# schatty/oprl

Measured on AMD Instinct MI355X. Metric: learner gradient steps/sec, DDPG batch=256 walker-walk, higher is better.
Workload: dtype f32 (exact-fp32 MFMA)

## Files before the change

oprl_amd/csrc/fused_ddpg.hip:

```cpp
#include <cstddef>
#include <mutex>
#include <type_traits>
#include "kernels.h"
#include "philox.h"
#include "replay_index.h"
#include "batch_rows.h"
#include "slice_head.h"
#include "tp4.h"
#include "dw_body.h"
#include "dw_tile_x2.h"

namespace oprl { constexpr bool kDwTileX2 = true; constexpr bool kMergedTile64 = true; }

namespace oprl {


__device__ __forceinline__ bool cluster_on_one_xcd(const DdpgArgs& A) {
  const int xcc = __builtin_amdgcn_s_getreg((3 << 11) | 20) & 15;
  return A.xcd_local != 0 && ((int)gridDim.x & 7) == 0 && xcc == ((int)blockIdx.x & 7);
}
__global__ void k_xcc_probe(int* out) {
  if (threadIdx.x == 0) out[blockIdx.y * gridDim.x + blockIdx.x] = __builtin_amdgcn_s_getreg((3 << 11) | 20) & 15;
}

// ... 893 lines not shown
  long long* trace;
  const float* pb1_32 = nullptr;
  unsigned mS = 0, mA = 0;
};
template <class P, class KA = DwKArgs, bool PF = true, bool GE = false>
__device__ __forceinline__ int ddpg_phase2m_body(const DdpgArgs& A, const KA* D, int by_in, const PassCtx& cx) {
  static_assert((P::kX2 || GE) && kDwTileX2, "the merged phase 2: PrecX2 learners; with the unit-seed rows (k_ddpg_chain) every arithmetic");
  extern __shared__ __attribute__((aligned(16))) float smem[];
  using LY = FusedLds<256>;
  constexpr int HB = kR * kWL4;
  constexpr int NMC = 8;
  const int B = A.B, S = A.S, Ad = A.A, tid = threadIdx.x;
  const int slice = blockIdx.x, row0 = slice * kR;
  const int y = by_in < 0 ? (int)blockIdx.y : by_in;
  const int yP = NMC, yT = yP + ((PF && A.prefetch_next) ? 1 : 0);
  if (y >= yT) {
    const int tile = (y - yT) * (int)gridDim.x + slice;
    if (tile >= dw_total(*D)) return -1;
    if (A.whole) {
      wait_flags(A.w_flags, 4 * (int)gridDim.x, cx.epoch, A.err, (KERN_PHASE2 << 8) | SITE_DW_GATE);
      __syncthreads();
    }
    return tile;
  }
  float* xa = smem + LY::xa;
  if (PF && y == yP) {
    float* xb = smem + LY::xb;
    float* rS = smem + LY::misc;
    float* dS = rS + kR;
    int* meta = reinterpret_cast<int*>(dS + 2 * kR);
    int* endsS = reinterpret_cast<int*>(smem + LY::misc + 96);
    load_batch(A.next, row0, B, S, Ad, xa, xb, rS, dS, meta, endsS);
    __syncthreads();
    store_rows(xa, kX0Ld, const_cast<float*>(A.next.s), S, S, row0, B);
    store_rows(xb, kX0Ld, const_cast<float*>(A.next.s2), S, S, row0, B);
    for (int idx = tid; idx < kR * Ad; idx += kThreads) {
      const int row = idx / Ad, col = idx - row * Ad, gr = row0 + row;
      if (gr < B) const_cast<float*>(A.next.a)[(size_t)gr * Ad + col] = xa[row * kX0Ld + S + col];
    }
    if (tid < kR && row0 + tid < B) {
      const_cast<float*>(A.next.r)[row0 + tid] = rS[tid];
      const_cast<float*>(A.next.d)[row0 + tid] = dS[tid];
    }
    return -1;
  }
  float* h1 = smem + LY::h;
  float* h2 = h1 + HB;
  float* g2 = h2 + HB;
  float* Wl = g2 + HB;
  float* outS = smem + LY::out;
  float* auxS = smem + LY::aux;
  float* duS = smem + LY::aux2;
  float* scr = smem + LY::scr;
  float* w3s = smem + LY::misc + 96;
  static_assert(2 * HB >= 2 * 8 * 512, "the shard fits the two spare hidden buffers");
  static_assert(kMaxEnds >= kDuLd * 256, "W3 fits the ends table's area");
  Tp tp{y, NMC, A.xbuf + (size_t)slice * kTpStages * A.xnc * kTpBlk, cx.tag, 0,
        A.err, KERN_PHASE2 << 8, A.debug_expire == (int)SITE_CLUSTER ? 0 : kTpSpin};
  tp.local = GE && cluster_on_one_xcd(A);
  const bool lead = tp.c == 0;
  const int c = tp.c;
  const int lane = tid & 63, wave = tid >> 6, i = lane & 15, kk = lane >> 4;
  long long* const trace = cx.trace;
  int n_stamp = 0;
  auto stamp = [&]() {
    if (kTraceOn && trace != nullptr && (tid & 63) == 0 && (tid == 0 || slice == 0) && lead && n_stamp < kTraceStamps) {
      const int slot = tid == 0 ? slice : 16 + (tid >> 6);
      long long* tr = trace + ((size_t)slot * kTraceStamps + n_stamp) * 2;
      tr[0] = (long long)__builtin_readcyclecounter();
      tr[1] = (long long)wall_clock64();
    }
    ++n_stamp;
  };
  stamp();
  const Tp3Store nostore{nullptr, nullptr, nullptr, nullptr, 0};
  BiasOv cbo;
  if (A.whole) {
    wait_flags(A.w_flags, 4 * (int)gridDim.x, cx.epoch, A.err, (KERN_PHASE2 << 8) | SITE_DW_GATE);
    __syncthreads();
  }
  stamp();
  {
    const float* p0 = A.aX[0]; const float* p3 = A.pi; const int ld0 = A.aldx0;
    asm volatile("" :: "s"(p0), "s"(p3), "s"(ld0));
  }
  const float* wsrc = ((P::kBf16 && cx.pb1_32 != nullptr) ? cx.pb1_32 : A.actor.pb[1]) + (size_t)c * 2 * 16 * 256;
  f32x4 wv[2];
#pragma unroll
  for (int q = 0; q < 2; ++q) wv[q] = ld4c(wsrc + ((size_t)q * kThreads + tid) * 4);
  const int hr = tid >> 6, hc = (tid & 63) * 4;
  f32x4 hv = f32x4{0.f, 0.f, 0.f, 0.f};
  if (row0 + hr < B) hv = ld4c(A.aX[2] + (size_t)(row0 + hr) * kW4 + hc);
  f32x4 w3q = f32x4{0.f, 0.f, 0.f, 0.f};
  if ((tid >> 6) < Ad) w3q = ld4c(cx.w3 + (size_t)tid * 4);
  const int et = (tid >> 8) & 1, er = (tid >> 4) & 15, ec = tid & 15;
  float m1 = 0.f;
  if (!GE && tid < 512 && row0 + er < B) m1 = ldc(A.aX[1] + (size_t)(row0 + er) * kW4 + 32 * c + 16 * et + ec);
  f32x4 gm1 = f32x4{0.f, 0.f, 0.f, 0.f};
  if constexpr (GE) {
#pragma unroll
    for (int r = 0; r < 4; ++r)
      if (row0 + 4 * kk + r < B) gm1[r] = ldc(A.aX[1] + (size_t)(row0 + 4 * kk + r) * kW4 + 32 * c + 16 * (wave & 1) + i);
  }
  const int rs_ = GE ? row_div(tid, cx.mS) : tid / S, cs_ = tid - rs_ * S;
  const bool oks = tid < kR * S && row0 + rs_ < B;
  const float vs = oks ? ldc(A.aX[0] + (size_t)(row0 + rs_) * A.aldx0 + cs_) : 0.f;
  const int tid2 = tid + kThreads;
  const int rs2_ = GE ? row_div(tid2, cx.mS) : tid2 / S, cs2_ = tid2 - rs2_ * S;
  const bool oks2 = tid2 < kR * S && row0 + rs2_ < B;
  const float vs2 = oks2 ? ldc(A.aX[0] + (size_t)(row0 + rs2_) * A.aldx0 + cs2_) : 0.f;
  const int rp_ = GE ? row_div(tid, cx.mA) : tid / Ad, cp_ = tid - rp_ * Ad;
  const bool okp = tid < kR * Ad && row0 + rp_ < B;
  const float vp = okp ? ldc(A.pi + (size_t)(row0 + rp_) * Ad + cp_) : 0.f;
  lds_zero(xa, kR * kX0Ld);
  lds_zero(auxS, kR * kOutLd);
  __syncthreads();
  if (tid < kR * S) xa[rs_ * kX0Ld + cs_] = vs;
  if (tid2 < kR * S) xa[rs2_ * kX0Ld + cs2_] = vs2;
  if (tid < kR * Ad) xa[rp_ * kX0Ld + S + cp_] = vp;
#pragma unroll
  for (int q = 0; q < 2; ++q) *reinterpret_cast<f32x4*>(Wl + ((size_t)q * kThreads + tid) * 4) = wv[q];
  if (tid < kDuLd * 64) *reinterpret_cast<f32x4*>(w3s + (size_t)tid * 4) = w3q;
  const unsigned mbits = (hv[0] > 0.f ? 1u : 0u) | (hv[1] > 0.f ? 2u : 0u) | (hv[2] > 0.f ? 4u : 0u) | (hv[3] > 0.f ? 8u : 0u) |
                         (m1 > 0.f ? 16u : 0u);
  stamp();
  if constexpr (GE && !P::kX2) {
    float* mS = h1;
    *reinterpret_cast<f32x4*>(mS + hr * kWL4 + hc) = f32x4{(mbits & 1u) ? 1.f : 0.f, (mbits & 2u) ? 1.f : 0.f, (mbits & 4u) ? 1.f : 0.f, (mbits & 8u) ? 1.f : 0.f};
    __syncthreads();
    const int t1 = wave & 1, j = wave >> 1;
    if (j < Ad) {
      f32x4 acc0 = f32x4{0.f, 0.f, 0.f, 0.f}, acc1 = acc0;
#pragma unroll 4
      for (int sx = 0; sx < 16; ++sx) {
        const f32x4 b4 = ld4(Wl + ((size_t)t1 * 16 + sx) * 256 + lane * 4);
        const f32x4 a4 = ld4(mS + i * kWL4 + 16 * sx + 4 * kk) * ld4(w3s + j * 256 + 16 * sx + 4 * kk);
        if (sx & 1) { mac4(a4, b4, acc1); } else { mac4(a4, b4, acc0); }
      }
#pragma unroll
      for (int r = 0; r < 4; ++r)
        if (row0 + 4 * kk + r < B)
          st_ag(A.gu + ((size_t)j * B + row0 + 4 * kk + r) * kW4 + 32 * c + 16 * t1 + i, gm1[r] > 0.f ? acc0[r] + acc1[r] : 0.f);
    }
    stamp();
  }
  if constexpr (GE && P::kX2) {
    typedef _Float16 f16x4 __attribute__((ext_vector_type(4)));
    _Float16* mH = reinterpret_cast<_Float16*>(h1);
    _Float16* wH = reinterpret_cast<_Float16*>(h1 + 2048);
    _Float16* wL = reinterpret_cast<_Float16*>(h1 + 2048 + 1024);
    float* sJ = h1 + 2048 + 2048;
    static_assert(HB >= 2048 + 2048 + 16, "masks and the output layer's planes fit one hidden buffer");
    {
      const int l = tid & 63, ws_ = l >> 3, half_ = (l >> 2) & 1, kq_ = l & 3;
      const int off = ((ws_ * 4 + kq_) * 8) + 4 * half_;
      union { f16x4 v; unsigned short b[4]; } mk;
#pragma unroll
      for (int t = 0; t < 4; ++t) mk.b[t] = ((mbits >> t) & 1u) ? 0xffffu : 0u;
      *reinterpret_cast<f16x4*>(mH + hr * 256 + off) = mk.v;
      if ((tid >> 6) < kDuLd) {
        float m = fmaxf(fmaxf(fabsf(w3q[0]), fabsf(w3q[1])), fmaxf(fabsf(w3q[2]), fabsf(w3q[3])));
        m = wave_max(m);
        const float sj = P::a_scale(m);
        f16x8 hi8, lo8;
        x2_split8(w3q * sj, f32x4{0.f, 0.f, 0.f, 0.f}, hi8, lo8);
        *reinterpret_cast<f16x4*>(wH + (tid >> 6) * 256 + off) = __builtin_shufflevector(hi8, hi8, 0, 1, 2, 3);
        *reinterpret_cast<f16x4*>(wL + (tid >> 6) * 256 + off) = __builtin_shufflevector(lo8, lo8, 0, 1, 2, 3);
        if (l == 0) sJ[tid >> 6] = sj;
      }
    }
    __syncthreads();
    const int t1 = wave & 1, j = wave >> 1;
    if (j < Ad) {
      f32x4 acc = f32x4{0.f, 0.f, 0.f, 0.f};
      typedef unsigned u32x4v __attribute__((ext_vector_type(4)));
#pragma unroll
      for (int ws = 0; ws < 8; ++ws) {
        const float* bw = Wl + ((size_t)t1 * 8 + ws) * 512 + lane * 4;
        const f16x8 bh = __builtin_bit_cast(f16x8, ld4(bw)), bl = __builtin_bit_cast(f16x8, ld4(bw + 256));
        const u32x4v mk = *reinterpret_cast<const u32x4v*>(mH + i * 256 + (ws * 4 + kk) * 8);
        const u32x4v h4 = *reinterpret_cast<const u32x4v*>(wH + j * 256 + (ws * 4 + kk) * 8);
        const u32x4v l4 = *reinterpret_cast<const u32x4v*>(wL + j * 256 + (ws * 4 + kk) * 8);
        const f16x8 ah = __builtin_bit_cast(f16x8, h4 & mk), al = __builtin_bit_cast(f16x8, l4 & mk);
        acc = __builtin_amdgcn_mfma_f32_16x16x32_f16(al, bh, acc, 0, 0, 0);
        acc = __builtin_amdgcn_mfma_f32_16x16x32_f16(ah, bl, acc, 0, 0, 0);
        acc = __builtin_amdgcn_mfma_f32_16x16x32_f16(ah, bh, acc, 0, 0, 0);
      }
      const float un = PrecX2::kOut / sJ[j];
#pragma unroll
      for (int r = 0; r < 4; ++r)
        if (row0 + 4 * kk + r < B)
          st_ag(A.gu + ((size_t)j * B + row0 + 4 * kk + r) * kW4 + 32 * c + 16 * t1 + i, gm1[r] > 0.f ? acc[r] * un : 0.f);
    }
    stamp();
  }
  if (A.whole) {
    if (tid < A.n_ct && A.debug_expire != 102) {
      bool ok = false;
      for (int spin = 0; spin < kTpSpin && !ok; ++spin) {
        ok = (unsigned)(__hip_atomic_load(A.ct_done + tid, __ATOMIC_RELAXED, __HIP_MEMORY_SCOPE_AGENT) >> 32) == cx.epoch;
        if (!ok) __builtin_amdgcn_s_sleep(1);
      }
      if (!ok) report_expired(A.err, (KERN_PHASE2 << 8) | SITE_DW_GATE);
    }
    __syncthreads();
    cbo.b0 = cx.cb[0]; cbo.b1 = cx.cb[1]; cbo.b2 = cx.cb[2];
  }
  if constexpr (GE) {
    asm volatile("s_waitcnt vmcnt(0)" ::: "memory");
    __syncthreads();
    if (tid == 0)
      __hip_atomic_store(A.gu_flags + slice * NMC + c, (unsigned long long)cx.epoch << 32, __ATOMIC_RELAXED, __HIP_MEMORY_SCOPE_AGENT);
  }
  stamp();
  float* qsum = nullptr;
  if (A.partials_a != nullptr && lead) {
    qsum = A.partials_a + slice * 4 + 1;
    if (tid == 0) { A.partials_a[slice * 4 + 0] = 0.f; A.partials_a[slice * 4 + 2] = 0.f; }
  }
  tp4_scalar_fb<typename std::conditional<GE, Coh<P>, P>::type, NMC>(A.critic, xa, h1, h2, g2, outS, scr, tp, nostore, row0, B, -A.inv_B, S, Ad, auxS, stamp, qsum, cbo);
  stamp();
  if (lead && okp) {
    const float du = auxS[rp_ * kOutLd + cp_] * (1.f - vp * vp);
    granule_put(A.du_granules + (size_t)(row0 + rp_) * kDuLd + cp_, cx.epoch, du);
    A.adY[2][(size_t)(row0 + rp_) * A.alddo + cp_] = du;
  }
  if constexpr (GE) { stamp(); return -1; }
  if constexpr (P::kX2 && !GE) {
    f32x4 gq = f32x4{0.f, 0.f, 0.f, 0.f};
    const bool row_in = row0 + hr < B;
#pragma unroll
    for (int j = 0; j < kDuLd; ++j) {
      float d = 0.f;
      if (j < Ad && row_in) {
        const float pv = xa[hr * kX0Ld + S + j];
        d = auxS[hr * kOutLd + j] * (1.f - pv * pv);
      }
      gq += ld4(w3s + j * 256 + hc) * d;
    }
#pragma unroll
    for (int t = 0; t < 4; ++t) gq[t] = ((mbits >> t) & 1u) != 0u ? gq[t] : 0.f;
    float m = fmaxf(fmaxf(fabsf(gq[0]), fabsf(gq[1])), fmaxf(fabsf(gq[2]), fabsf(gq[3])));
    m = wave_max(m);
    const float sr = P::a_scale(m);
    *reinterpret_cast<f32x4*>(h1 + hr * kWL4 + hc) = gq * sr;
    if (lane == 0) duS[hr] = PrecX2::kOut / sr;
  }
  __syncthreads();
  {
    const int t1 = wave & 1, ws = wave >> 1;
    const float* hrow = h1 + i * kWL4 + 4 * kk;
    const float* bw = Wl + ((size_t)t1 * 8 + ws) * 512 + lane * 4;
    const FragX2 bf{ld4(bw), ld4(bw + 256)};
    const f32x4 un = ld4(duS + 4 * kk);
    f32x4 acc = f32x4{0.f, 0.f, 0.f, 0.f};
    PrecX2::mma3(ld4(hrow + 32 * ws), ld4(hrow + 32 * ws + 16), bf, acc);
    float* o = scr + wave * 256;
#pragma unroll
    for (int r = 0; r < 4; ++r) o[(4 * kk + r) * 16 + i] = acc[r] * un[r];
  }
  __syncthreads();
  if (tid < 512 && row0 + er < B) {
    float v = 0.f;
#pragma unroll
    for (int ws = 0; ws < 8; ++ws) v += scr[(2 * ws + et) * 256 + er * 16 + ec];
    v = (mbits & 16u) != 0u ? v : 0.f;
    granule_put(const_cast<unsigned long long*>(A.g1_granules) + ((size_t)(2 * c + et) * B + row0 + er) * 16 + ec, cx.epoch, v);
  }
  stamp();
  return -1;
}

template <class P>
__global__ __launch_bounds__(kThreads) void k_ddpg_phase2_dw(const DdpgArgs A, const DwKArgs D) {
  const DwKArgs* Dp = (const DwKArgs*)((const char*)__builtin_amdgcn_kernarg_segment_ptr() + kMergedDwOffset);
  const PassCtx cx{A.epoch, A.cluster_tag, A.w3_snap, {A.critic_b16[0], A.critic_b16[1], A.critic_b16[2]}, A.trace};
  ddpg_tile<P, DwKArgs>(Dp, ddpg_phase2m_body<P>(A, Dp, -1, cx), 2);
}

constexpr size_t kWholeDcOffset = (sizeof(DdpgArgs) + alignof(DwKArgs4) - 1) / alignof(DwKArgs4) * alignof(DwKArgs4);
constexpr size_t kWholeDaOffset = (kWholeDcOffset + sizeof(DwKArgs4) + alignof(DwKArgs4) - 1) / alignof(DwKArgs4) * alignof(DwKArgs4);

__device__ __forceinline__ void chain_wait2(const unsigned long long* f0, int n0, const unsigned long long* f1, int n1,
                                            const unsigned long long* f2, int n2, unsigned tag, unsigned* err, unsigned code) {
  const int k = (int)threadIdx.x;
  const unsigned long long* f = k < n0 ? f0 + k : (k < n0 + n1 ? f1 + (k - n0) : (k < n0 + n1 + n2 ? f2 + (k - n0 - n1) : nullptr));
  if (f != nullptr) {
    bool ok = false;
    for (int spin = 0; spin < kTpSpin && !ok; ++spin) {
      ok = (unsigned)(__hip_atomic_load(f, __ATOMIC_RELAXED, __HIP_MEMORY_SCOPE_AGENT) >> 32) == tag;
      if (!ok) __builtin_amdgcn_s_sleep(1);
    }
    if (!ok) report_expired(err, code);
  }
  __syncthreads();
}

constexpr size_t kChainCOffset = (kWholeDaOffset + sizeof(DwKArgs4) + alignof(ChainArgs) - 1) / alignof(ChainArgs) * alignof(ChainArgs);
__device__ __forceinline__ int chain_row(int y, int order) {
  if (y >= 16 || order == 0) return y;
  if (order == 1) return y < 4 ? y + 8 : (y < 12 ? y - 4 : y);
  if (order == 2) return y < 8 ? y + 8 : y - 8;
  return y < 8 ? y : (y < 12 ? y + 4 : y - 4);
}

template <class P>
__global__ __launch_bounds__(kThreads) void k_ddpg_chain(const DdpgArgs A, const DwKArgs4 Dc, const DwKArgs4 Da, const ChainArgs C_) {
  static_assert(kDwTileX2, "the chain launch runs the 16 x 64 tiles of dw_tile_x2.h");
  extern __shared__ __attribute__((aligned(16))) float smem[];
  const char* ka = (const char*)__builtin_amdgcn_kernarg_segment_ptr();
  const DwKArgs4* Dcp = (const DwKArgs4*)(ka + kWholeDcOffset);
  const DwKArgs4* Dap = (const DwKArgs4*)(ka + kWholeDaOffset);
  const ChainArgs& C = *(const ChainArgs*)(ka + kChainCOffset);
  using LY = FusedLds<256>;
  constexpr int HB = kR * kWL4;
  const int slices = (int)gridDim.x, slice = (int)blockIdx.x;
  const int u = (int)blockIdx.z, yy = chain_row((int)blockIdx.y, C.order);
  const int B = A.B, S = A.S, Ad = A.A, tid = threadIdx.x, row0 = slice * kR;
  const unsigned ep = A.epoch + (unsigned)u;
  const unsigned tag1 = A.cluster_tag + 2u * (unsigned)u, tag2 = tag1 + 1u;
  const int tc = Dcp->tile_end[kDwFusedItems - 1], ta = Dap->tile_end[kDwFusedItems - 1];
  const int par = u & 1;
  float* xa = smem + LY::xa;
  float* xb = smem + LY::xb;
  float* h1 = smem + LY::h;
  float* h2 = h1 + HB;
  float* outS = smem + LY::out;
  float* scr = smem + LY::scr;
  float* rS = smem + LY::misc;
  float* dS = rS + kR;
  float* yS = dS + kR;
  int* meta = reinterpret_cast<int*>(yS + kR);
  int* endsS = reinterpret_cast<int*>(smem + LY::misc + 96);
  const int role = yy < 8 ? 0 : (yy < 12 ? 1 : (yy < 16 ? 2 : 3));
  const int member = yy < 8 ? yy : (yy < 16 ? (yy - 8) & 3 : 1);
  const bool lead = member == 0;
  const int spin = A.debug_expire == (int)SITE_CLUSTER ? 0 : kTpSpin;
  const bool traced = kTraceOn && A.trace != nullptr && u == C.trace_u;
  int n_stamp = 0;
  auto stamp = [&]() {
    if (traced && role < 3 && (tid & 63) == 0 && (tid == 0 || slice == 0) && lead && n_stamp < kTraceStamps) {
      const int slot = tid == 0 ? slice : 16 + (tid >> 6);
      long long* tr = A.trace + (((size_t)role * 64 + slot) * kTraceStamps + n_stamp) * 2;
      tr[0] = (long long)__builtin_readcyclecounter();
      tr[1] = (long long)wall_clock64();
    }
    ++n_stamp;
  };
  stamp();

  if (u > 0 && role == 0) chain_wait2(C.pf_done + slice, 1, nullptr, 0, nullptr, 0, ep - 1u, A.err, (KERN_PHASE1 << 8) | SITE_DW_GATE);
  if (u > 0 && role != 0) chain_wait2(C.ct_fin, tc, C.at_fin, role == 1 ? 0 : ta, C.pf_done + slice, role == 3 ? 0 : 1, ep - 1u, A.err, (KERN_PHASE1 << 8) | SITE_DW_GATE);
  if (role == 3) {
  } else if (u == 0 && C.first_gather) {
    load_batch(A.src, row0, B, S, Ad, xa, xb, rS, dS, meta, endsS);
  } else {
    const float* ps = par ? C.set1[0] : C.set0[0]; const float* pa = par ? C.set1[1] : C.set0[1];
    const float* pr = par ? C.set1[2] : C.set0[2]; const float* pd = par ? C.set1[3] : C.set0[3];
    const float* ps2 = par ? C.set1[4] : C.set0[4];
    lds_zero(xa, 2 * kR * kX0Ld);
    __syncthreads();
    load_rows_c<true>(xa, kX0Ld, 0, ps, S, S, row0, B, C.mS);
    load_rows_c<true>(xa, kX0Ld, S, pa, Ad, Ad, row0, B, C.mA);
    load_rows_c<true>(xb, kX0Ld, 0, ps2, S, S, row0, B, C.mS);
    if (tid < kR) {
      const int gr = row0 + tid;
      rS[tid] = gr < B ? ldc(pr + gr) : 0.f;
      dS[tid] = gr < B ? ldc(pd + gr) : 0.f;
    }
  }
  stamp();
  if (u > 0 && role == 0) {
    __syncthreads();
    chain_wait2(C.ct_fin, tc, C.at_fin, ta, nullptr, 0, ep - 1u, A.err, (KERN_PHASE1 << 8) | SITE_DW_GATE);
  }
  stamp();
  const Tp3Store nostore{nullptr, nullptr, nullptr, nullptr, 0};
  auto bias_of = [&](int which) {
    BiasOv bo;
    if (u > 0) { bo.b0 = C.b16[which][0]; bo.b1 = C.b16[which][1]; bo.b2 = C.b16[which][2]; }
    return bo;
  };

  if (role == 0) {
    Tp tp{member, 8, A.xbuf + (size_t)slice * kTpStages * A.xnc * kTpBlk, tag1, 0, A.err, KERN_PHASE1 << 8, spin};
    tp.local = cluster_on_one_xcd(A);
    tp4_forward<Coh<P>, 8>(A.actor_t, xb, h1, h2, outS, scr, tp, nostore, row0, B, stamp, bias_of(1));
    for (int idx = tid; idx < kR * Ad; idx += kThreads) {
      const int row = row_div(idx, C.mA), col = idx - row * Ad, gr = row0 + row;
      xb[row * kX0Ld + S + col] = gr < B ? tanhf(outS[row * kOutLd + col]) : 0.f;
    }
    unsigned long long gq[4] = {0ull, 0ull, 0ull, 0ull};
    float qb = 0.f;
    int hook_n = 0;
    const unsigned long long* gq_src = C.qp + (size_t)slice * 64 + (tid & (kR - 1));
    auto hook = [&]() {
      stamp();
      if (++hook_n == 2) {
#pragma unroll
        for (int m = 0; m < 4; ++m) gq[m] = __hip_atomic_load(gq_src + m * kR, __ATOMIC_RELAXED, __HIP_MEMORY_SCOPE_AGENT);
        qb = ldc(u > 0 ? C.b16[2][2] : A.critic.b[2]);
      }
    };
    tp4_forward<Coh<P>, 8>(A.critic_t, xb, h1, h2, outS, scr, tp, nostore, row0, B, hook, bias_of(3));
    if (lead && tid < 64) {
      const int gr = row0 + tid;
      const bool row_ok = tid < kR && gr < B;
      const float qn = row_ok ? outS[tid * kOutLd] : 0.f;
      const float y = row_ok ? rS[tid] + ((1.f - dS[tid]) * A.gamma) * qn : 0.f;
      const int lim = A.debug_expire == (int)SITE_TD_TARGET ? 0 : (1 << 20);
      float q = 0.f;
      if (row_ok) {
        bool ok = lim > 0;
#pragma unroll
        for (int m = 0; m < 4; ++m) ok = ok && (unsigned)(gq[m] >> 32) == ep;
        if (A.debug_expire == 101) ok = true;
        for (int sp = 0; sp < lim && !ok; ++sp) {
#pragma unroll
          for (int m = 0; m < 4; ++m) gq[m] = __hip_atomic_load(gq_src + m * kR, __ATOMIC_RELAXED, __HIP_MEMORY_SCOPE_AGENT);
          ok = true;
#pragma unroll
          for (int m = 0; m < 4; ++m) ok = ok && (unsigned)(gq[m] >> 32) == ep;
          if (!ok) __builtin_amdgcn_s_sleep(1);
        }
        if (!ok) report_expired(A.err, (KERN_PHASE1 << 8) | SITE_TD_TARGET);
        float qs = 0.f;
#pragma unroll
        for (int m = 0; m < 4; ++m) qs += __uint_as_float((unsigned)gq[m]);
        q = ok ? qs + qb : __builtin_nanf("");
        const float seed = 2.f * (q - y) * A.inv_B;
        A.cdY[2][(size_t)gr * A.clddo] = seed;
        __hip_atomic_store(A.y_granules + gr, ((unsigned long long)ep << 32) | (unsigned long long)__float_as_uint(seed),
                           __ATOMIC_RELAXED, __HIP_MEMORY_SCOPE_AGENT);
        if (A.y_out != nullptr) A.y_out[gr] = y;
        if (A.q_out != nullptr) A.q_out[gr] = q;
      }
      if (A.partials_c != nullptr) {
        float v[3] = {row_ok ? (q - y) * (q - y) : 0.f, row_ok ? q : 0.f, row_ok ? y : 0.f};
#pragma unroll
        for (int k = 0; k < 3; ++k) {
          const float sum = row16_sum(v[k]);
          if (tid == 0) A.partials_c[(size_t)slice * 4 + k] = sum;
        }
      }
    }
    stamp();
    __syncthreads();
    int by2 = (int)blockIdx.y, u2 = (int)blockIdx.z;
    asm volatile("" : "+s"(by2), "+s"(u2));
    const PassCtx cx{A.epoch + (unsigned)u2, A.cluster_tag + 2u * (unsigned)u2 + 1u, C.w3buf[u2 & 1], {C.b16[2][0], C.b16[2][1], C.b16[2][2]},
                     (kTraceOn && u2 == C.trace_u) ? A.trace2 : nullptr, A.actor_pb1_f32, C.mS, C.mA};
    (void)ddpg_phase2m_body<P, DwKArgs4, false, true>(A, Dap, chain_row(by2, C.order), cx);
    return;
  }

  if (role == 1) {
    Tp tp{member, 4, A.xbuf + ((size_t)1 * slices + slice) * kTpStages * A.xnc * kTpBlk, tag1, 0, A.err, KERN_PHASE1 << 8, spin};
    tp.local = cluster_on_one_xcd(A);
    const Tp3Store st{A.cX[1], A.cX[2], A.cdY[1], A.cdY[0], A.cdY0_stride, B, true};
    if (lead) {
      __syncthreads();
      for (int idx = tid; idx < kR * (S + Ad); idx += kThreads) {
        const int row = row_div(idx, C.mSA), col = idx - row * (S + Ad), gr = row0 + row;
        if (gr < B) __hip_atomic_store(A.cX[0] + (size_t)gr * A.cldx0 + col, xa[row * kX0Ld + col], __ATOMIC_RELAXED, __HIP_MEMORY_SCOPE_AGENT);
      }
    }
    const QPart qp{C.qp + (size_t)slice * 64, ep};
    tp4_scalar_fb<Coh<P>>(A.critic, xa, h1, h2, h1 + 2 * HB, outS, scr, tp, st, row0, B, 1.f, 0, 0, nullptr, stamp, nullptr, bias_of(2), qp);
    asm volatile("s_waitcnt vmcnt(0)" ::: "memory");
    __syncthreads();
    if (tid == 0)
      __hip_atomic_store(A.gate_flags + slice * 4 + member, (unsigned long long)ep << 32, __ATOMIC_RELAXED, __HIP_MEMORY_SCOPE_AGENT);
    stamp();
  } else if (role == 2) {
    Tp tp{member, 4, A.xbuf + ((size_t)2 * slices + slice) * kTpStages * A.xnc * kTpBlk, tag1, 0, A.err, KERN_PHASE1 << 8, spin};
    tp.local = cluster_on_one_xcd(A);
    const Tp3Store st{A.aX[1], A.aX[2], nullptr, nullptr, 0, 0, true};
    tp4_forward<Coh<P>>(A.actor, xa, h1, h2, outS, scr, tp, st, row0, B, stamp, bias_of(0));
    if (lead) {
      for (int idx = tid; idx < kR * Ad; idx += kThreads) {
        const int row = row_div(idx, C.mA), col = idx - row * Ad, gr = row0 + row;
        if (gr < B) st_ag(A.pi + (size_t)gr * Ad + col, tanhf(outS[row * kOutLd + col]));
      }
      store_rows_wt<true>(xa, kX0Ld, A.aX[0], A.aldx0, S, row0, B, C.mS);
      if (u == 0 && slice == 0)
        for (int idx = tid * 4; idx < Ad * kW4; idx += kThreads * 4)
          st16_wt(C.w3buf[0], idx, ld4(A.w3_src + idx));
    }
    stamp();
    asm volatile("s_waitcnt vmcnt(0)" ::: "memory");
    __syncthreads();
    if (tid == 0)
      __hip_atomic_store(A.w_flags + slice * 4 + member, (unsigned long long)ep << 32, __ATOMIC_RELAXED, __HIP_MEMORY_SCOPE_AGENT);
  }
  __syncthreads();
  int by2 = (int)blockIdx.y, bx2 = (int)blockIdx.x, nx2 = (int)gridDim.x, u2 = (int)blockIdx.z;
  asm volatile("" : "+s"(by2), "+s"(bx2), "+s"(nx2), "+s"(u2));
  const int y2 = chain_row(by2, C.order);
  const int wg2 = y2 < 16 ? ((y2 >= 12) ? 4 * nx2 : 0) + bx2 * 4 + ((y2 - 8) & 3) : 8 * nx2 + (y2 - 16) * nx2 + bx2;
  const int n_bc = 8 * nx2;
  const unsigned ep2 = A.epoch + (unsigned)u2;

  {
    const int p = n_bc + (C.rows - 16) * nx2 - 1 - wg2;
    if (p >= 0 && p < nx2 && (u2 + 1 < C.n_upd || C.pf_last)) {
      const int par2 = u2 & 1;
      BatchSrc nx = A.next;
      nx.s = par2 ? C.set0[0] : C.set1[0]; nx.a = par2 ? C.set0[1] : C.set1[1]; nx.r = par2 ? C.set0[2] : C.set1[2];
      nx.d = par2 ? C.set0[3] : C.set1[3]; nx.s2 = par2 ? C.set0[4] : C.set1[4];
      nx.counter = A.next.counter + (unsigned long long)u2;
      prefetch_rows_src<true>(nx, A.S, A.A, A.B, p, smem);
      asm volatile("s_waitcnt vmcnt(0)" ::: "memory");
      __syncthreads();
      if (threadIdx.x == 0)
        __hip_atomic_store(C.pf_done + p, (unsigned long long)ep2 << 32, __ATOMIC_RELAXED, __HIP_MEMORY_SCOPE_AGENT);
    }
  }
  {
    const int tile = wg2 < Dcp->tile_end[kDwFusedItems - 1] ? wg2 : -1;
    if (tile >= 0) {
      DwX2Ovr ov;
      ov.chain = &C; ov.u = u2;
      dw_tile_x2<DwKArgs4, P>(*Dcp, smem, tile, 1, ov);
    }
  }
  {
    int by3 = (int)blockIdx.y, bx3 = (int)blockIdx.x, nx3 = (int)gridDim.x, u3 = (int)blockIdx.z;
    asm volatile("" : "+s"(by3), "+s"(bx3), "+s"(nx3), "+s"(u3));
    const int y3 = chain_row(by3, C.order);
    const int wg3 = y3 < 16 ? ((y3 >= 12) ? 4 * nx3 : 0) + bx3 * 4 + ((y3 - 8) & 3) : 8 * nx3 + (y3 - 16) * nx3 + bx3;
    const int tile = wg3 < Dap->tile_end[kDwFusedItems - 1] ? wg3 : -1;
    if (tile >= 0) {
      __syncthreads();
      wait_flags(A.w_flags, 4 * nx3, A.epoch + (unsigned)u3, A.err, (KERN_PHASE2 << 8) | SITE_DW_GATE);
      if (u3 > 0 && threadIdx.x == kThreads - 1) {
        bool ok = false;
        for (int sp = 0; sp < kTpSpin && !ok; ++sp) {
          ok = (unsigned)(__hip_atomic_load(C.at_fin + tile, __ATOMIC_RELAXED, __HIP_MEMORY_SCOPE_AGENT) >> 32) == A.epoch + (unsigned)u3 - 1u;
          if (!ok) __builtin_amdgcn_s_sleep(2);
        }
        if (!ok) report_expired(A.err, (KERN_PHASE2 << 8) | SITE_DW_GATE);
      }
      __syncthreads();
      DwX2Ovr ov;
      ov.chain = &C; ov.u = u3;
      dw_tile_x2<DwKArgs4, P>(*Dap, smem, tile, 2, ov);
    }
  }
}

static_assert(FusedLds<256>::total >= kDwLdsFloats && FusedLds<256>::total >= DwLds<16>::floats && FusedLds<256>::total >= DwX2Lds::floats, "a tile workgroup fits the phase kernels' LDS");
bool fused_x2_tiles() { return kDwTileX2; }
bool fused_tile64_all() { return kDwTileX2 && kMergedTile64; }

size_t fused_ddpg_lds_bytes() { return sizeof(float) * FusedLds<256>::total; }
size_t fused_xbuf_granules_per_cluster(int nc) { return (size_t)kTpStages * nc * kTpBlk; }

bool xcd_map_ok() {
  static std::mutex mu;
  static int known[16] = {0};
  int dev = 0;
  if (hipGetDevice(&dev) != hipSuccess) return false;
  std::lock_guard<std::mutex> lk(mu);
  int& k = known[dev & 15];
  if (k != 0) return k > 0;
  k = -1;
  int* d = nullptr;
  if (hipMalloc(&d, 256 * sizeof(int)) != hipSuccess) return false;
  bool ok = true;
  int h[256];
  for (int rep = 0; rep < 3 && ok; ++rep) {
    ok = hipMemset(d, 0xff, 256 * sizeof(int)) == hipSuccess;
    if (ok) hipLaunchKernelGGL(k_xcc_probe, dim3(16, 16), dim3(64), 0, 0, d);
    ok = ok && hipMemcpy(h, d, sizeof h, hipMemcpyDeviceToHost) == hipSuccess;
    for (int b = 0; b < 256 && ok; ++b) ok = h[b] == (b & 7);
  }
  (void)hipFree(d);
  if (ok) k = 1;
  return ok;
}

hipError_t init_fused_attrs() {
  const void* ks[] = {reinterpret_cast<const void*>(&k_ddpg_phase1<256, false, false>),
                      reinterpret_cast<const void*>(&k_ddpg_phase1<256, true, false>),
                      reinterpret_cast<const void*>(&k_ddpg_phase1<256, true, true>),
                      reinterpret_cast<const void*>(&k_ddpg_phase2<256, false, false>),
                      reinterpret_cast<const void*>(&k_ddpg_phase2<256, true, false>),
                      reinterpret_cast<const void*>(&k_ddpg_phase2<256, true, true>),
                      reinterpret_cast<const void*>(&k_ddpg_phase1<256, true, false, PrecBF16>),
                      reinterpret_cast<const void*>(&k_ddpg_phase1<256, true, true, PrecBF16>),
                      reinterpret_cast<const void*>(&k_ddpg_phase2<256, true, false, PrecBF16>),
                      reinterpret_cast<const void*>(&k_ddpg_phase2<256, true, true, PrecBF16>),
                      reinterpret_cast<const void*>(&k_ddpg_phase1<256, true, false, PrecX2>),
                      reinterpret_cast<const void*>(&k_ddpg_phase1<256, true, true, PrecX2>),
                      reinterpret_cast<const void*>(&k_ddpg_phase2<256, true, false, PrecX2>),
                      reinterpret_cast<const void*>(&k_ddpg_phase2<256, true, true, PrecX2>),
                      reinterpret_cast<const void*>(&k_ddpg_phase1_group<256, false, false>),
                      reinterpret_cast<const void*>(&k_ddpg_phase2_group<256, false, false>),
                      reinterpret_cast<const void*>(&k_ddpg_phase1_group<256, true, false, PrecF32>),
                      reinterpret_cast<const void*>(&k_ddpg_phase2_group<256, true, false, PrecF32>),
                      reinterpret_cast<const void*>(&k_ddpg_phase1_group<256, true, false, PrecBF16>),
                      reinterpret_cast<const void*>(&k_ddpg_phase2_group<256, true, false, PrecBF16>),
                      reinterpret_cast<const void*>(&k_ddpg_phase1_group<256, true, false, PrecX2>),
                      reinterpret_cast<const void*>(&k_ddpg_phase2_group<256, true, false, PrecX2>),
                      reinterpret_cast<const void*>(&k_ddpg_phase1_group<256, true, false, PrecF32, false>),
                      reinterpret_cast<const void*>(&k_ddpg_phase1_group<256, true, false, PrecBF16, false>),
                      reinterpret_cast<const void*>(&k_ddpg_phase1_group<256, true, false, PrecX2, false>),
                      reinterpret_cast<const void*>(&k_ddpg_phase1_group<256, true, true, PrecF32, false>),
                      reinterpret_cast<const void*>(&k_ddpg_phase1_group<256, true, true, PrecBF16, false>),
                      reinterpret_cast<const void*>(&k_ddpg_phase1_group<256, true, true, PrecX2, false>),
                      reinterpret_cast<const void*>(&k_ddpg_phase2_group<256, true, true, PrecF32>),
                      reinterpret_cast<const void*>(&k_ddpg_phase2_group<256, true, true, PrecBF16>),
                      reinterpret_cast<const void*>(&k_ddpg_phase2_group<256, true, true, PrecX2>),
                      reinterpret_cast<const void*>(&k_ddpg_phase1<256, true, false, PrecF32, true>),
                      reinterpret_cast<const void*>(&k_ddpg_phase2<256, true, false, PrecF32, true>),
                      reinterpret_cast<const void*>(&k_ddpg_phase1<256, true, false, PrecX2, true>),
                      reinterpret_cast<const void*>(&k_ddpg_phase2<256, true, false, PrecX2, true>),
                      reinterpret_cast<const void*>(&k_ddpg_phase1_dw<PrecF32>),
                      reinterpret_cast<const void*>(&k_ddpg_phase1_dw<PrecBF16>),
                      reinterpret_cast<const void*>(&k_ddpg_phase1_dw<PrecX2>),
                      reinterpret_cast<const void*>(&k_ddpg_phase1_dw<PrecX2, true>),
                      reinterpret_cast<const void*>(&k_ddpg_phase1_dw<PrecF32, false, true>),
                      reinterpret_cast<const void*>(&k_ddpg_phase1_dw<PrecBF16, false, true>),
                      reinterpret_cast<const void*>(&k_ddpg_phase1_dw<PrecX2, false, true>),
                      reinterpret_cast<const void*>(&k_ddpg_phase2_dw<PrecX2>),
                      reinterpret_cast<const void*>(&k_ddpg_chain<PrecX2>),
                      reinterpret_cast<const void*>(&k_ddpg_chain<PrecF32>),
                      reinterpret_cast<const void*>(&k_ddpg_chain<PrecBF16>),
                      reinterpret_cast<const void*>(&k_ddpg_phase1_rt2<false, PrecF32>),
                      reinterpret_cast<const void*>(&k_ddpg_phase1_rt2<false, PrecX2>),
                      reinterpret_cast<const void*>(&k_ddpg_phase1_rt2<false, PrecBF16>),
                      reinterpret_cast<const void*>(&k_ddpg_phase1_rt2<true, PrecF32>),
                      reinterpret_cast<const void*>(&k_ddpg_phase1_rt2<true, PrecX2>),
                      reinterpret_cast<const void*>(&k_ddpg_phase1_rt2<true, PrecBF16>)};
  for (const void* k : ks) {
    hipError_t e = hipFuncSetAttribute(k, hipFuncAttributeMaxDynamicSharedMemorySize, 160 * 1024);
    if (e != hipSuccess) return e;
  }
  return hipSuccess;
}

bool fused_ddpg_is_lean(const DdpgArgs& a);
template <class P>
static void launch_p1_group_lean(const DdpgArgs& a0, dim3 grid, const DdpgArgs* batch_dev, hipStream_t st) {
  const dim3 blk(kThreads);
  const size_t lds = fused_ddpg_lds_bytes();
  if (a0.sac) hipLaunchKernelGGL((k_ddpg_phase1_group<256, true, true, P, false>), grid, blk, lds, st, batch_dev);
  else if (a0.n_critics == 2) hipLaunchKernelGGL((k_ddpg_phase1_group<256, true, false, P, false>), grid, blk, lds, st, batch_dev);
  else hipLaunchKernelGGL((k_ddpg_phase1_group<256, true, false, P, true>), grid, blk, lds, st, batch_dev);
}
template <class P>
static void launch_p2_group_lean(const DdpgArgs& a0, dim3 grid, const DdpgArgs* batch_dev, hipStream_t st) {
  const dim3 blk(kThreads);
  const size_t lds = fused_ddpg_lds_bytes();
  if (a0.sac) hipLaunchKernelGGL((k_ddpg_phase2_group<256, true, true, P>), grid, blk, lds, st, batch_dev);
  else hipLaunchKernelGGL((k_ddpg_phase2_group<256, true, false, P>), grid, blk, lds, st, batch_dev);
}
hipError_t launch_ddpg_phase1_group(const DdpgArgs& a0, const DdpgArgs* batch_dev, int n, hipStream_t st) {
  if (a0.merged || a0.wide || a0.whole || a0.twin_split || a0.prefetch_p1 || (a0.sac && a0.n_critics != 2)) return hipErrorInvalidValue;
  dim3 grid((a0.B + kR - 1) / kR, (2 + a0.n_critics) * a0.nc, n);
  if (a0.nc == 4 && fused_ddpg_is_lean(a0)) {
    if (a0.x2) launch_p1_group_lean<PrecX2>(a0, grid, batch_dev, st);
    else if (a0.bf16) launch_p1_group_lean<PrecBF16>(a0, grid, batch_dev, st);
    else launch_p1_group_lean<PrecF32>(a0, grid, batch_dev, st);
    return hipGetLastError();
  }
  if (a0.nc != 1 || a0.bf16 || a0.x2 || a0.sac || a0.n_critics != 1) return hipErrorInvalidValue;
  grid = dim3((a0.B + kR - 1) / kR, 1, 3 * n);
  hipLaunchKernelGGL((k_ddpg_phase1_group<256, false, false>), grid, dim3(kThreads), fused_ddpg_lds_bytes(), st, batch_dev);
  return hipGetLastError();
}
hipError_t launch_ddpg_phase2_group(const DdpgArgs& a0, const DdpgArgs* batch_dev, int n, hipStream_t st) {
  if (a0.merged || a0.wide || a0.whole || a0.p2_pair || (a0.sac && a0.n_critics != 2)) return hipErrorInvalidValue;
  const dim3 grid((a0.B + kR - 1) / kR, a0.nc + (a0.prefetch_next ? 1 : 0), n);
  if (a0.nc == 4 && fused_ddpg_is_lean(a0)) {
    if (a0.x2) launch_p2_group_lean<PrecX2>(a0, grid, batch_dev, st);
    else if (a0.bf16) launch_p2_group_lean<PrecBF16>(a0, grid, batch_dev, st);
    else launch_p2_group_lean<PrecF32>(a0, grid, batch_dev, st);
    return hipGetLastError();
  }
  if (a0.nc != 1 || a0.bf16 || a0.x2 || a0.sac || a0.n_critics != 1) return hipErrorInvalidValue;
  hipLaunchKernelGGL((k_ddpg_phase2_group<256, false, false>), grid, dim3(kThreads), fused_ddpg_lds_bytes(), st, batch_dev);
  return hipGetLastError();
}

static bool lean_ok(const DdpgArgs& a) { return fused_ddpg_is_lean(a); }
bool fused_ddpg_is_lean(int nc, int no_lean, int S, int A, bool sac) {
  return nc == 4 && !no_lean && tp4_shape_ok(256, S + A, 1) && tp4_shape_ok(256, S, sac ? 2 * A : A);
}
bool fused_ddpg_is_lean(const DdpgArgs& a) { return fused_ddpg_is_lean(a.nc, a.no_lean, a.S, a.A, a.sac != 0); }

static_assert(kDuLd <= kSmallDivMaxD, "the chain launch's action sizes are narrow-exchange divisors");
static_assert((16 * kMaxS0 + 63) / 64 <= kSmallDivMaxD && kW4 / 64 <= kSmallDivMaxD, "the lean shapes' fan-ins are tile divisors");
static bool narrow8_ok(const DdpgArgs& a) { return a.A >= 1 && a.A <= kSmallDivMaxD; }
template <class KA>
static bool tiles64_ok(const KA& d) {
  if (d.n_items < 1 || d.n_items > KA::kItems) return false;
  if (d.tile_end[d.n_items - 1] >= kSmallDivMaxN) return false;
  for (int j = 0; j < d.n_items; ++j)
    if (d.items[j].K < 1 || (d.items[j].K + kDwX2TileK - 1) / kDwX2TileK > kSmallDivMaxD) return false;
  return true;
}

hipError_t launch_ddpg_phase1_dw(const DdpgArgs& a, const DwKArgs& d, hipStream_t st) {
  const bool wide = (a.wide & 1) != 0;
  if ((wide && !narrow8_ok(a)) || (kMergedTile64 && !tiles64_ok(d))) return hipErrorInvalidValue;
  if (!lean_ok(a) || a.sac || a.n_critics < 1 || a.n_critics > 2 || (a.merged & 1) == 0 || (wide && (!a.x2 || a.xnc < 8 || a.n_critics != 1))) return hipErrorInvalidValue;
  const int slices = (a.B + kR - 1) / kR;
  const int tiles = d.tile_end[kDwMaxItems - 1];
  const dim3 grid(slices, (2 + a.n_critics) * a.nc + (wide ? 4 : 0) + (tiles + slices - 1) / slices + (a.prefetch_p1 ? 1 : 0));
  if (a.n_critics == 2) {
    if (a.seed2_granules == nullptr) return hipErrorInvalidValue;
    if (a.x2) hipLaunchKernelGGL((k_ddpg_phase1_dw<PrecX2, false, true>), grid, dim3(kThreads), fused_ddpg_lds_bytes(), st, a, d);
    else if (a.bf16) hipLaunchKernelGGL((k_ddpg_phase1_dw<PrecBF16, false, true>), grid, dim3(kThreads), fused_ddpg_lds_bytes(), st, a, d);
    else hipLaunchKernelGGL((k_ddpg_phase1_dw<PrecF32, false, true>), grid, dim3(kThreads), fused_ddpg_lds_bytes(), st, a, d);
    return hipGetLastError();
  }
  if (a.x2 && wide) hipLaunchKernelGGL((k_ddpg_phase1_dw<PrecX2, true>), grid, dim3(kThreads), fused_ddpg_lds_bytes(), st, a, d);
  else if (a.x2) hipLaunchKernelGGL((k_ddpg_phase1_dw<PrecX2>), grid, dim3(kThreads), fused_ddpg_lds_bytes(), st, a, d);
  else if (a.bf16) hipLaunchKernelGGL((k_ddpg_phase1_dw<PrecBF16>), grid, dim3(kThreads), fused_ddpg_lds_bytes(), st, a, d);
  else hipLaunchKernelGGL((k_ddpg_phase1_dw<PrecF32>), grid, dim3(kThreads), fused_ddpg_lds_bytes(), st, a, d);
  return hipGetLastError();
}

hipError_t launch_ddpg_phase2_dw(const DdpgArgs& a, const DwKArgs& d, hipStream_t st) {
  if (!lean_ok(a) || a.sac || !a.x2 || !kDwTileX2 || (a.merged & 2) == 0 || (a.wide & 2) == 0 || a.xnc < 8 || a.A > kDuLd || a.B > 256)
    return hipErrorInvalidValue;
  if (!narrow8_ok(a) || !tiles64_ok(d)) return hipErrorInvalidValue;
  const int slices = (a.B + kR - 1) / kR;
  const int tiles = d.tile_end[kDwMaxItems - 1];
  const dim3 grid(slices, 8 + (a.prefetch_next ? 1 : 0) + (tiles + slices - 1) / slices);
  hipLaunchKernelGGL((k_ddpg_phase2_dw<PrecX2>), grid, dim3(kThreads), fused_ddpg_lds_bytes(), st, a, d);
  return hipGetLastError();
}

hipError_t launch_ddpg_chain(const DdpgArgs& a, const DwKArgs4& dc, const DwKArgs4& da, const ChainArgs& c, hipStream_t st) {
  if (!lean_ok(a) || a.sac || (a.bf16 && a.actor_pb1_f32 == nullptr) || !kDwTileX2 || a.n_critics != 1 || !a.whole || (a.merged & 3) != 3 || (a.wide & 3) != 3 ||
      a.xnc < 8 || a.A > kDuLd || a.B > 256 || a.prefetch_next || a.prefetch_p1 || c.n_upd < 1 || c.n_upd > kChainMax)
    return hipErrorInvalidValue;
  const int slices = (a.B + kR - 1) / kR;
  const int tc = dc.tile_end[kDwFusedItems - 1], ta = da.tile_end[kDwFusedItems - 1];
  if (tc + ta + 1 > kThreads) return hipErrorInvalidValue;
  const int mt = tc > ta ? tc : ta;
  const int rows = 16 + chain_tile_rows(mt, slices);
  if (c.rows != rows) return hipErrorInvalidValue;
  if (!narrow8_ok(a) || !tiles64_ok(dc) || !tiles64_ok(da)) return hipErrorInvalidValue;
  if (!row_div_ok(a.S + a.A) || c.mS != row_div_magic(a.S) || c.mA != row_div_magic(a.A) || c.mSA != row_div_magic(a.S + a.A)) return hipErrorInvalidValue;
  const dim3 grid(slices, rows, c.n_upd);
  if (a.x2) hipLaunchKernelGGL((k_ddpg_chain<PrecX2>), grid, dim3(kThreads), fused_ddpg_lds_bytes(), st, a, dc, da, c);
  else if (a.bf16) hipLaunchKernelGGL((k_ddpg_chain<PrecBF16>), grid, dim3(kThreads), fused_ddpg_lds_bytes(), st, a, dc, da, c);
  else hipLaunchKernelGGL((k_ddpg_chain<PrecF32>), grid, dim3(kThreads), fused_ddpg_lds_bytes(), st, a, dc, da, c);
  return hipGetLastError();
}

hipError_t launch_ddpg_phase1(const DdpgArgs& a, hipStream_t st) {
  const int slices = (a.B + kR - 1) / kR;
  const dim3 blk(kThreads);
  const size_t lds = fused_ddpg_lds_bytes();
  const int pf = a.prefetch_p1 ? 1 : 0;
  if ((a.wide & 1) != 0) {
    if (!lean_ok(a) || a.sac || a.bf16 || a.n_critics != 1 || a.xnc < 8 || !narrow8_ok(a)) return hipErrorInvalidValue;
    const dim3 grid(slices, a.nc + 8 + a.nc + pf);
    if (a.x2) hipLaunchKernelGGL((k_ddpg_phase1<256, true, false, PrecX2, true>), grid, blk, lds, st, a);
    else hipLaunchKernelGGL((k_ddpg_phase1<256, true, false, PrecF32, true>), grid, blk, lds, st, a);
    return hipGetLastError();
  }
  if (a.rt2) {
    if (!lean_ok(a) || a.nc != 4 || (slices & 15) != 0 || pf || a.merged != 0) return hipErrorInvalidValue;
    if (a.rt2 == 2 && (!a.sac || a.twin_split || !a.do_actor)) return hipErrorInvalidValue;
    const dim3 g2(slices, 2 * a.n_critics + (a.rt2 == 2 ? 1 : 2) * a.nc);
    const size_t l2 = std::max(lds, sizeof(float) * (size_t)FusedLdsB2::total);
    if (a.sac) {
      if (a.x2) hipLaunchKernelGGL((k_ddpg_phase1_rt2<true, PrecX2>), g2, blk, l2, st, a);
      else if (a.bf16) hipLaunchKernelGGL((k_ddpg_phase1_rt2<true, PrecBF16>), g2, blk, l2, st, a);
      else hipLaunchKernelGGL((k_ddpg_phase1_rt2<true, PrecF32>), g2, blk, l2, st, a);
    } else {
      if (a.x2) hipLaunchKernelGGL((k_ddpg_phase1_rt2<false, PrecX2>), g2, blk, l2, st, a);
      else if (a.bf16) hipLaunchKernelGGL((k_ddpg_phase1_rt2<false, PrecBF16>), g2, blk, l2, st, a);
      else hipLaunchKernelGGL((k_ddpg_phase1_rt2<false, PrecF32>), g2, blk, l2, st, a);
    }
    return hipGetLastError();
  }
  const dim3 grid(slices, (2 + a.n_critics) * a.nc + pf);
  if (a.bf16 || a.x2) {
    if (!lean_ok(a)) return hipErrorInvalidValue;
    if (a.x2 && a.sac) hipLaunchKernelGGL((k_ddpg_phase1<256, true, true, PrecX2>), grid, blk, lds, st, a);
    else if (a.x2) hipLaunchKernelGGL((k_ddpg_phase1<256, true, false, PrecX2>), grid, blk, lds, st, a);
    else if (a.sac) hipLaunchKernelGGL((k_ddpg_phase1<256, true, true, PrecBF16>), grid, blk, lds, st, a);
    else hipLaunchKernelGGL((k_ddpg_phase1<256, true, false, PrecBF16>), grid, blk, lds, st, a);
  } else if (a.sac) {
    if (!lean_ok(a)) return hipErrorInvalidValue;
    hipLaunchKernelGGL((k_ddpg_phase1<256, true, true>), grid, blk, lds, st, a);
  } else if (lean_ok(a)) {
    hipLaunchKernelGGL((k_ddpg_phase1<256, true, false>), grid, blk, lds, st, a);
  } else {
    hipLaunchKernelGGL((k_ddpg_phase1<256, false, false>), grid, blk, lds, st, a);
  }
  return hipGetLastError();
}

hipError_t launch_ddpg_phase2(const DdpgArgs& a, hipStream_t st) {
  const int slices = (a.B + kR - 1) / kR;
  const dim3 blk(kThreads);
  const size_t lds = fused_ddpg_lds_bytes();
  if ((a.wide & 2) != 0) {
    if (!lean_ok(a) || a.sac || a.bf16 || a.xnc < 8 || !narrow8_ok(a)) return hipErrorInvalidValue;
    const dim3 grid(slices, 8 + (a.prefetch_next ? 1 : 0));
    if (a.x2) hipLaunchKernelGGL((k_ddpg_phase2<256, true, false, PrecX2, true>), grid, blk, lds, st, a);
    else hipLaunchKernelGGL((k_ddpg_phase2<256, true, false, PrecF32, true>), grid, blk, lds, st, a);
    return hipGetLastError();
  }
  const dim3 grid(slices, a.nc * ((a.sac && a.p2_pair) ? 2 : 1) + (a.prefetch_next ? 1 : 0));
  if (a.bf16 || a.x2) {
    if (!lean_ok(a)) return hipErrorInvalidValue;
    if (a.x2 && a.sac) hipLaunchKernelGGL((k_ddpg_phase2<256, true, true, PrecX2>), grid, blk, lds, st, a);
    else if (a.x2) hipLaunchKernelGGL((k_ddpg_phase2<256, true, false, PrecX2>), grid, blk, lds, st, a);
    else if (a.sac) hipLaunchKernelGGL((k_ddpg_phase2<256, true, true, PrecBF16>), grid, blk, lds, st, a);
    else hipLaunchKernelGGL((k_ddpg_phase2<256, true, false, PrecBF16>), grid, blk, lds, st, a);
  } else if (a.sac) {
    if (!lean_ok(a)) return hipErrorInvalidValue;
    hipLaunchKernelGGL((k_ddpg_phase2<256, true, true>), grid, blk, lds, st, a);
  } else if (lean_ok(a)) {
    hipLaunchKernelGGL((k_ddpg_phase2<256, true, false>), grid, blk, lds, st, a);
  } else {
    hipLaunchKernelGGL((k_ddpg_phase2<256, false, false>), grid, blk, lds, st, a);
  }
  return hipGetLastError();
}

}
```

Baseline: 35680.

## Prefetch chain batch rows into registers and overlap with TP forward start

In the fp32 chain kernel, roles 1 and 2 now issue global loads of the next batch's state/action rows into registers before the tensor-parallel forward starts. They write those rows into LDS, and for the critic lead also to cX[0], through a hook passed to tp4_forward/tp4_scalar_fb. Role 0 now loads only its own next-state and reward/done inputs. The aim is to hide gather latency behind the cross-workgroup exchange instead of doing a zero/load/sync before the forward. The cost is extra register pressure and a dependency on the tp4 functions accepting the new callback, whose headers are not shown.

After: 35600. About the same (-0.2%).

```diff
diff --git a/oprl_amd/csrc/fused_ddpg.hip b/oprl_amd/csrc/fused_ddpg.hip
--- a/oprl_amd/csrc/fused_ddpg.hip
+++ b/oprl_amd/csrc/fused_ddpg.hip
@@ -1219,6 +1219,41 @@
   if (order == 1) return y < 4 ? y + 8 : (y < 12 ? y - 4 : y);
   if (order == 2) return y < 8 ? y + 8 : y - 8;
   return y < 8 ? y : (y < 12 ? y + 4 : y - 4);
+}
+
+constexpr int kRowsPer = (kR * kX0Ld + kThreads - 1) / kThreads;
+__device__ __forceinline__ void chain_rows_req(float (&rv)[kRowsPer], const float* ps, const float* pa, int S, int na, int row0, int B) {
+  const int tid = threadIdx.x;
+#pragma unroll
+  for (int j = 0; j < kRowsPer; ++j) {
+    const int idx = min(tid + j * kThreads, kR * kX0Ld - 1);
+    const int row = idx / kX0Ld, col = idx - row * kX0Ld, gr = row0 + row;
+    const bool is_s = gr < B && col < S, is_a = gr < B && col >= S && col < S + na;
+    const float* src = ps;
+    if (is_s) src = ps + (size_t)gr * S + col;
+    if (is_a) src = pa + (size_t)gr * na + (col - S);
+    const float x = ldc(src);
+    rv[j] = (is_s || is_a) ? x : 0.f;
+  }
+  __builtin_amdgcn_sched_barrier(0);
+}
+__device__ __forceinline__ void chain_rows_put(float* xa, const float (&rv)[kRowsPer]) {
+  const int tid = threadIdx.x;
+#pragma unroll
+  for (int j = 0; j < kRowsPer; ++j) {
+    const int idx = tid + j * kThreads;
+    if (idx < kR * kX0Ld) xa[idx] = rv[j];
+  }
+}
+__device__ __forceinline__ void chain_rows_out(float* G, int ldg, int k, const float (&rv)[kRowsPer], int row0, int B) {
+  const int tid = threadIdx.x;
+#pragma unroll
+  for (int j = 0; j < kRowsPer; ++j) {
+    const int idx = tid + j * kThreads;
+    const int row = idx / kX0Ld, col = idx - row * kX0Ld, gr = row0 + row;
+    if (idx < kR * kX0Ld && gr < B && col < k)
+      __hip_atomic_store(G + (size_t)gr * ldg + col, rv[j], __ATOMIC_RELAXED, __HIP_MEMORY_SCOPE_AGENT);
+  }
 }
 
 template <class P>
@@ -1268,7 +1303,27 @@
 
   if (u > 0 && role == 0) chain_wait2(C.pf_done + slice, 1, nullptr, 0, nullptr, 0, ep - 1u, A.err, (KERN_PHASE1 << 8) | SITE_DW_GATE);
   if (u > 0 && role != 0) chain_wait2(C.ct_fin, tc, C.at_fin, role == 1 ? 0 : ta, C.pf_done + slice, role == 3 ? 0 : 1, ep - 1u, A.err, (KERN_PHASE1 << 8) | SITE_DW_GATE);
-  if (role == 3) {
+  constexpr bool OV = !P::kBf16;
+  const float* ps = nullptr; const float* pa = nullptr;
+  if constexpr (OV) {
+    const bool gather0 = u == 0 && C.first_gather;
+    ps = par ? C.set1[0] : C.set0[0]; pa = par ? C.set1[1] : C.set0[1];
+    const float* pr = par ? C.set1[2] : C.set0[2]; const float* pd = par ? C.set1[3] : C.set0[3];
+    const float* ps2 = par ? C.set1[4] : C.set0[4];
+    if (role == 3) {
+    } else if (gather0) {
+      load_batch(A.src, row0, B, S, Ad, xa, xb, rS, dS, meta, endsS);
+    } else if (role == 0) {
+      lds_zero(xb, kR * kX0Ld);
+      __syncthreads();
+      load_rows_c<true>(xb, kX0Ld, 0, ps2, S, S, row0, B, C.mS);
+      if (tid < kR) {
+        const int gr = row0 + tid;
+        rS[tid] = gr < B ? ldc(pr + gr) : 0.f;
+        dS[tid] = gr < B ? ldc(pd + gr) : 0.f;
+      }
+    }
+  } else if (role == 3) {
   } else if (u == 0 && C.first_gather) {
     load_batch(A.src, row0, B, S, Ad, xa, xb, rS, dS, meta, endsS);
   } else {
@@ -1286,6 +1341,7 @@
       dS[tid] = gr < B ? ldc(pd + gr) : 0.f;
     }
   }
+  const bool rows_bc = OV && !(u == 0 && C.first_gather);
   stamp();
   if (u > 0 && role == 0) {
     __syncthreads();
@@ -1375,7 +1431,7 @@
     Tp tp{member, 4, A.xbuf + ((size_t)1 * slices + slice) * kTpStages * A.xnc * kTpBlk, tag1, 0, A.err, KERN_PHASE1 << 8, spin};
     tp.local = cluster_on_one_xcd(A);
     const Tp3Store st{A.cX[1], A.cX[2], A.cdY[1], A.cdY[0], A.cdY0_stride, B, true};
-    if (lead) {
+    if (lead && !rows_bc) {
       __syncthreads();
       for (int idx = tid; idx < kR * (S + Ad); idx += kThreads) {
         const int row = row_div(idx, C.mSA), col = idx - row * (S + Ad), gr = row0 + row;
@@ -1383,7 +1439,18 @@
       }
     }
     const QPart qp{C.qp + (size_t)slice * 64, ep};
-    tp4_scalar_fb<Coh<P>>(A.critic, xa, h1, h2, h1 + 2 * HB, outS, scr, tp, st, row0, B, 1.f, 0, 0, nullptr, stamp, nullptr, bias_of(2), qp);
+    if constexpr (OV) {
+      float rv[kRowsPer] = {};
+      if (rows_bc) chain_rows_req(rv, ps, pa, S, Ad, row0, B);
+      auto rows_pre = [&]() {
+        if (!rows_bc) return;
+        chain_rows_put(xa, rv);
+        if (lead) chain_rows_out(A.cX[0], A.cldx0, S + Ad, rv, row0, B);
+      };
+      tp4_scalar_fb<Coh<P>>(A.critic, xa, h1, h2, h1 + 2 * HB, outS, scr, tp, st, row0, B, 1.f, 0, 0, nullptr, stamp, nullptr, bias_of(2), qp, rows_pre);
+    } else {
+      tp4_scalar_fb<Coh<P>>(A.critic, xa, h1, h2, h1 + 2 * HB, outS, scr, tp, st, row0, B, 1.f, 0, 0, nullptr, stamp, nullptr, bias_of(2), qp);
+    }
     asm volatile("s_waitcnt vmcnt(0)" ::: "memory");
     __syncthreads();
     if (tid == 0)
@@ -1393,7 +1460,16 @@
     Tp tp{member, 4, A.xbuf + ((size_t)2 * slices + slice) * kTpStages * A.xnc * kTpBlk, tag1, 0, A.err, KERN_PHASE1 << 8, spin};
     tp.local = cluster_on_one_xcd(A);
     const Tp3Store st{A.aX[1], A.aX[2], nullptr, nullptr, 0, 0, true};
-    tp4_forward<Coh<P>>(A.actor, xa, h1, h2, outS, scr, tp, st, row0, B, stamp, bias_of(0));
+    if constexpr (OV) {
+      float rv[kRowsPer] = {};
+      if (rows_bc) chain_rows_req(rv, ps, ps, S, 0, row0, B);
+      auto rows_pre = [&]() {
+        if (rows_bc) chain_rows_put(xa, rv);
+      };
+      tp4_forward<Coh<P>>(A.actor, xa, h1, h2, outS, scr, tp, st, row0, B, stamp, bias_of(0), rows_pre);
+    } else {
+      tp4_forward<Coh<P>>(A.actor, xa, h1, h2, outS, scr, tp, st, row0, B, stamp, bias_of(0));
+    }
     if (lead) {
       for (int idx = tid; idx < kR * Ad; idx += kThreads) {
         const int row = row_div(idx, C.mA), col = idx - row * Ad, gr = row0 + row;
@@ -1470,6 +1546,7 @@
 bool fused_x2_tiles() { return kDwTileX2; }
 bool fused_tile64_all() { return kDwTileX2 && kMergedTile64; }
 
+static_assert(sizeof(float) * FusedLds<256>::total <= 160 * 1024, "the fused launches' dynamic LDS fits what init_fused_attrs grants");
 size_t fused_ddpg_lds_bytes() { return sizeof(float) * FusedLds<256>::total; }
 size_t fused_xbuf_granules_per_cluster(int nc) { return (size_t)kTpStages * nc * kTpBlk; }
 
```
